# bit-current/DistributedTraining

Measured on AMD Instinct MI355X. Metric: tokens/sec (whole node, all miners), GPT-2-small local-SGD, higher is better.
Workload: dtype bf16; 1 GPU; model=gpt2-small, global_batch=1024, seq_len=64, parallelism=local_sgd_dp1, merge_every=25, optimizer=fused AdamW (lr 5e-4, reference config)

## Files before the change

distributedtraining_amd/ops/__init__.py:

```python

from __future__ import annotations

import math
from typing import Optional

import torch
import torch.nn.functional as F

from . import droprng
from .backend import require_ext, use_hip

__all__ = [
    "layer_norm", "rms_norm", "gelu", "swiglu", "causal_attention",
    "qkv_attention", "linear", "mlp_gelu", "add_layer_norm",
    "add_rms_norm",
    "cross_entropy_loss", "lm_head_ce", "lm_head_loss",
    "embedding_fwd", "check_q_lo", "check_doc_start", "q_lo_inverse",
    "decode_attention", "rope", "adamw_step", "delta_sub", "axpy_",
    "weighted_merge",
    "grad_merge_weights", "has_nan", "l2norm",
    "grad_sumsq_blocks", "grad_sumsq_partials", "step_control",
    "adamw_step_guarded", "lr_schedule",
    "quantize_blockwise_int8", "dequantize_blockwise_int8",
    "topk_compress_blockwise",
    "dropout", "rng_tick",
]


import os as _os

_USE_BGRADB = _os.environ.get("DTA_LT_BGRADB", "0") == "1"

class _LinearFn(torch.autograd.Function):

    @staticmethod
    def forward(ctx, x, w, b):
        x2 = x.reshape(-1, x.shape[-1])
        ctx.save_for_backward(x2, w)
        ctx.has_b = b is not None
        ctx.xshape = x.shape
        ctx.wgrad = getattr(w, "main_grad", None)
        ctx.bgrad = getattr(b, "main_grad", None) if b is not None else None
        y = torch.addmm(b, x2, w.t()) if b is not None else x2.mm(w.t())
        return y.view(*x.shape[:-1], w.shape[0])

    @staticmethod
    def backward(ctx, dy):
        x2, w = ctx.saved_tensors
        dy2 = dy.reshape(-1, dy.shape[-1])
        if dy2.stride(-1) != 1:
            dy2 = dy2.contiguous()
        dx = dy2.mm(w).view(ctx.xshape)
        m = require_ext()
        if _USE_BGRADB and ctx.has_b and ctx.wgrad is not None:
            try:
                db = m.lt_wgrad_bgradb(dy2, x2, ctx.wgrad)
                return dx, None, db
            except RuntimeError:
                pass
        if ctx.wgrad is not None:
            ctx.wgrad.addmm_(dy2.t(), x2)
            dw = None
        else:
            dw = dy2.t().mm(x2)
        db = (_cast_grad(m.colsum(dy2, ctx.bgrad), w.dtype)
              if ctx.has_b else None)
        return dx, dw, db


def linear(x: torch.Tensor, w: torch.Tensor,
           b: Optional[torch.Tensor] = None) -> torch.Tensor:
    if use_hip(x):
        rows = x.numel() // x.shape[-1]
        if rows <= 4 and not torch.is_grad_enabled() and _gemv_wins(rows, w):
            x2 = x.reshape(rows, x.shape[-1])
            if not x2.is_contiguous():
                x2 = x2.contiguous()
            y = require_ext().gemv(
                x2, w, b if b is not None
                else torch.empty(0, dtype=w.dtype, device=w.device))
            return y.view(*x.shape[:-1], w.shape[0])
        return _LinearFn.apply(x, w, b)
    return F.linear(x, w, b)


def _gemv_wins(rows: int, w: torch.Tensor) -> bool:
    if w.shape[1] % 8 != 0:
        return False
    numel = w.shape[0] * w.shape[1]
    return numel < (20_000_000 if rows == 1 else 5_000_000)


_lt_fused_shape_ok: dict = {}


class _FusedMLPFn(torch.autograd.Function):

    @staticmethod
    def forward(ctx, x, w1, b1, w2, b2):
        m = require_ext()
        x2 = x.reshape(-1, x.shape[-1])
        h, aux = m.lt_linear_gelu_fwd(x2.contiguous(), w1, b1)
        y = torch.addmm(b2, h, w2.t())
        ctx.save_for_backward(x2, w1, w2, h, aux)
        ctx.xshape = x.shape
        ctx.w1grad = getattr(w1, "main_grad", None)
        ctx.w2grad = getattr(w2, "main_grad", None)
        ctx.b2grad = getattr(b2, "main_grad", None)
        return y.view(*x.shape[:-1], w2.shape[0])

    @staticmethod
    def backward(ctx, dy):
        m = require_ext()
        x2, w1, w2, h, aux = ctx.saved_tensors
        dy2 = dy.reshape(-1, dy.shape[-1])
        if dy2.stride(-1) != 1:
            dy2 = dy2.contiguous()
        db2 = _cast_grad(m.colsum(dy2, ctx.b2grad), w2.dtype)
        if ctx.w2grad is not None:
            ctx.w2grad.addmm_(dy2.t(), h)
            dw2 = None
        else:
            dw2 = dy2.t().mm(h)
        dh_pre, db1 = m.lt_dgrad_dgelu_bgrad(dy2, w2, aux)
        if ctx.w1grad is not None:
            ctx.w1grad.addmm_(dh_pre.t(), x2)
            dw1 = None
        else:
            dw1 = dh_pre.t().mm(x2)
        dx = dh_pre.mm(w1).view(ctx.xshape)
        return dx, dw1, db1, dw2, db2


_MLP_NODE = _os.environ.get("DTA_MLP_NODE", "1") != "0"


def mlp_node_enable(on: bool) -> bool:
    global _MLP_NODE
    prev, _MLP_NODE = _MLP_NODE, bool(on)
    return prev


class _MLPGeluFn(torch.autograd.Function):

    @staticmethod
    def forward(ctx, x, w1, b1, w2, b2):
        m = require_ext()
        x2 = x.reshape(-1, x.shape[-1])
        pre = torch.addmm(b1, x2, w1.t())
        h = m.gelu_fwd(pre)
        y = torch.addmm(b2, h, w2.t())
        ctx.save_for_backward(x2, w1, w2, pre, h)
        ctx.xshape = x.shape
        ctx.grads = tuple(getattr(t, "main_grad", None)
                          for t in (w1, b1, w2, b2))
        return y.view(*x.shape[:-1], w2.shape[0])

    @staticmethod
    def backward(ctx, dy):
        m = require_ext()
        x2, w1, w2, pre, h = ctx.saved_tensors
        w1g, b1g, w2g, b2g = ctx.grads
        dy2 = dy.reshape(-1, dy.shape[-1])
        if dy2.stride(-1) != 1:
            dy2 = dy2.contiguous()
        dh = dy2.mm(w2)
        if w2g is not None:
            w2g.addmm_(dy2.t(), h)
            dw2 = None
        else:
            dw2 = dy2.t().mm(h)
        db2 = _cast_grad(m.colsum(dy2, b2g), w2.dtype)
        dh_pre, db1 = m.gelu_bwd_colsum(dh, pre, b1g)
        del dh
        dx = dh_pre.mm(w1).view(ctx.xshape)
        if w1g is not None:
            w1g.addmm_(dh_pre.t(), x2)
            dw1 = None
        else:
            dw1 = dh_pre.t().mm(x2)
        return dx, dw1, _cast_grad(db1, w1.dtype), dw2, db2


def mlp_gelu(x: torch.Tensor, w1: torch.Tensor, b1: torch.Tensor,
             w2: torch.Tensor, b2: torch.Tensor) -> torch.Tensor:
    if use_hip(x):
        rows = x.numel() // x.shape[-1]
        if rows <= 4 and not torch.is_grad_enabled():
            return linear(gelu(linear(x, w1, b1)), w2, b2)
        key = (rows, w1.shape[0], w1.shape[1])
        if _lt_fused_shape_ok.get(key, True):
            try:
                out = _FusedMLPFn.apply(x, w1, b1, w2, b2)
                _lt_fused_shape_ok[key] = True
                return out
            except RuntimeError as e:
                import logging
                logging.getLogger(__name__).warning(
                    "hipBLASLt epilogue MLP unavailable at M,N,K=%s (%s); "
                    "composed path", key, e)
                _lt_fused_shape_ok[key] = False
        if _MLP_NODE and all(t.dtype == torch.bfloat16
                             for t in (x, w1, b1, w2, b2)):
            return _MLPGeluFn.apply(x, w1, b1, w2, b2)
        return linear(gelu(linear(x, w1, b1)), w2, b2)
    return F.linear(F.gelu(F.linear(x, w1, b1), approximate="tanh"), w2, b2)


def _empty_like0(t):
    return t.new_empty(0)


def _rng0(t: torch.Tensor) -> torch.Tensor:
    return droprng.counter(t.device)


def _grad_out(fp32_grad, main_grad, dtype):
    if main_grad is not None:
        require_ext().accum_f32_into_bf16(main_grad, fp32_grad)
        return None
    return fp32_grad.to(dtype)


def _cast_grad(fp32_grad, dtype):
    return None if fp32_grad is None else fp32_grad.to(dtype)


def _cpu_drop(t: torch.Tensor, p: float, site: int) -> torch.Tensor:
    keep = droprng.elem_keep_mask(t.numel(), droprng.value(t.device), site, p)
    mask = torch.from_numpy(keep.astype("float32")).reshape(t.shape)
    return t * (mask * droprng.inv_keep(p)).to(t.dtype)


def _norm_fwd(x2, res, w, b, eps, site, p):
    m = require_ext()
    if b is None:
        y, rstd, s = m.rmsnorm_fwd(x2, res, w, eps, _rng0(x2), site, p)
        return y, (rstd,), s
    y, mean, rstd, s = m.layernorm_fwd(x2, res, w, b, eps, _rng0(x2), site, p)
    return y, (mean, rstd), s


def _norm_bwd(dy, ds, x2, w, stats, site, p, wg=None, bg=None):
    m = require_ext()
    if len(stats) == 1:
        dx, dw32, dres = m.rmsnorm_bwd(dy, ds, x2, w, *stats, _rng0(x2),
                                       site, p, wg)
        return dx, dw32, None, dres
    return m.layernorm_bwd(dy, ds, x2, w, *stats, _rng0(x2), site, p, wg, bg)


class _NormFn(torch.autograd.Function):
    @staticmethod
    def forward(ctx, x, w, b, eps):
        x2 = x.contiguous()
        y, stats, _ = _norm_fwd(x2.view(-1, x2.shape[-1]), _empty_like0(x2),
                                w, b, eps, 0, 0.0)
        ctx.save_for_backward(x2, w, *stats)
        ctx.wg = getattr(w, "main_grad", None)
# ... 975 lines not shown
```

distributedtraining_amd/ops/hip/bindings.cpp:

```cpp
#include <torch/extension.h>
#include <ATen/hip/HIPContext.h>

#include <algorithm>
#include <atomic>
#include <vector>

#include "dta_kernels.h"

namespace {

using torch::Tensor;

inline hipStream_t stream() {
  return at::hip::getCurrentHIPStream().stream();
}
inline const bf16_t* bfp(const Tensor& t) {
  return reinterpret_cast<const bf16_t*>(t.data_ptr());
}
inline bf16_t* bfp_mut(Tensor& t) {
  return reinterpret_cast<bf16_t*>(t.data_ptr());
}

void check_bf16(const Tensor& t, const char* name) {
  TORCH_CHECK(t.is_cuda(), name, " must be on GPU");
// ... 271 lines not shown
  }
  TORCH_CHECK(has_part || (max_norm <= 0.0 && !skip_nonfinite),
              "clipping and the non-finite skip need the norm partials");
  TORCH_CHECK(part.numel() <= (int64_t(1) << 30), "too many partials");
  TORCH_CHECK(schedule >= LR_CONSTANT && schedule <= LR_COSINE,
              "unknown schedule");
  TORCH_CHECK(warmup_steps >= 0 && warmup_steps < (int64_t(1) << 31) &&
                  total_steps >= 0 && total_steps < (int64_t(1) << 31),
              "warmup_steps / total_steps out of range");
  TORCH_CHECK(schedule == LR_CONSTANT || total_steps > warmup_steps,
              "linear / cosine need total_steps > warmup_steps");
  launch_step_ctl({has_part ? part.data_ptr<float>() : nullptr,
                   int(part.numel()), ctl_f.data_ptr<float>(),
                   ctl_i.data_ptr<int>(), beta1, beta2, float(max_norm),
                   skip_nonfinite ? 1 : 0, int(schedule), lr_max, min_lr,
                   int(warmup_steps), int(total_steps)},
                  stream());
}
void adamw_step_guarded(Tensor master, Tensor grad, Tensor m, Tensor v,
                        Tensor out_bf16, Tensor ctl_f, Tensor ctl_i,
                        double beta1, double beta2, double eps, double wd) {
  check_f32(master, "master"); check_f32(m, "m"); check_f32(v, "v");
  const bool gb = flat_grad_is_bf16(grad, "grad");
  const int64_t n = master.numel();
  TORCH_CHECK(grad.numel() == n && m.numel() == n && v.numel() == n,
              "master, grad, m and v must have one length");
  TORCH_CHECK(grad.device() == master.device() &&
                  m.device() == master.device() &&
                  v.device() == master.device(), "planes on one device");
  check_ctl(ctl_f, ctl_i, master);
  bf16_t* outp = nullptr;
  if (out_bf16.numel()) {
    check_bf16(out_bf16, "out_bf16");
    TORCH_CHECK(out_bf16.numel() == n && out_bf16.device() == master.device(),
                "out_bf16 must match master");
    outp = bfp_mut(out_bf16);
  }
  launch_adamw_guarded(master.data_ptr<float>(), grad.data_ptr(), gb,
                       m.data_ptr<float>(), v.data_ptr<float>(), outp,
                       ctl_f.data_ptr<float>(), ctl_i.data_ptr<int>(), beta1,
                       beta2, float(eps), float(wd), n, stream());
}

Tensor colsum(Tensor x, OptTensor dst) {
  check_bf16(x, "x");
  TORCH_CHECK(x.dim() == 2 && x.size(1) >= 1, "x must be [rows, cols]");
  const int64_t rows = x.size(0);
  const int cols = int(x.size(1));
  const int stripes = dta_colred_stripes(rows, cols);
  auto f32 = x.options().dtype(torch::kFloat32);
  auto part = torch::empty({stripes, dta_colred_ld(cols)}, f32);
  bf16_t* d = grad_dst(dst, cols, "dst");
  Tensor out = d ? Tensor() : torch::empty({cols}, f32);
  launch_colsum(bfp(x), part.data_ptr<float>(),
                d ? nullptr : out.data_ptr<float>(), d, rows, cols, stripes,
                stream());
  return out;
}

std::vector<Tensor> gelu_bwd_colsum(Tensor dy, Tensor x, OptTensor db_dst,
                                    int64_t stripes_arg) {
  check_bf16(x, "x"); check_bf16(dy, "dy");
  TORCH_CHECK(x.dim() == 2 && dy.sizes() == x.sizes(),
              "dy, x must be [rows, cols]");
  const int64_t rows = x.size(0);
  const int cols = int(x.size(1));
  if (cols % 8 != 0) {
    auto dx = gelu_bwd(dy, x);
    return {dx, colsum(dx, db_dst)};
  }
  const int stripes =
      stripes_arg > 0 ? int(std::min<int64_t>(stripes_arg, 65535))
                      : dta_gelu_colsum_stripes(rows, cols);
  auto f32 = x.options().dtype(torch::kFloat32);
  auto dx = torch::empty_like(x);
  auto part = torch::empty({stripes, cols}, f32);
  bf16_t* d = grad_dst(db_dst, cols, "db_dst");
  Tensor out = d ? Tensor() : torch::empty({cols}, f32);
  launch_gelu_bwd_colsum(bfp(dy), bfp(x), bfp_mut(dx),
                         part.data_ptr<float>(),
                         d ? nullptr : out.data_ptr<float>(), d, rows, cols,
                         stripes, stream());
  return {dx, out};
}

int merge_n_models(int64_t n) {
  TORCH_CHECK(n >= 1 && n <= DTA_MERGE_MAX_MODELS,
              "merge: 1 <= n_models <= ", DTA_MERGE_MAX_MODELS);
  return int(n);
}
int merge_n_segs(const Tensor& offsets) {
  TORCH_CHECK(offsets.dim() == 1 && offsets.numel() >= 2 &&
                  (offsets.scalar_type() == torch::kInt64 ||
                   offsets.scalar_type() == torch::kInt32),
              "offsets must be an int64 or int32 [n_segs + 1] tensor");
  TORCH_CHECK(offsets.numel() <= int64_t(DTA_MERGE_LDS_LIMIT / 8),
              "offsets do not fit the LDS budget of ", DTA_MERGE_LDS_LIMIT,
              " B");
  return int(offsets.numel() - 1);
}
Tensor merge_offsets(const Tensor& offsets, const Tensor& base) {
  return offsets.to(base.device(), torch::kInt64).contiguous();
}
Tensor merge_weights(const Tensor& W, const Tensor& base, int n_models,
                     int n_segs) {
  TORCH_CHECK(W.dim() == 2 && W.size(0) == n_models && W.size(1) == n_segs,
              "W must be [n_models, n_segs]");
  TORCH_CHECK(dta_merge_shmem(n_models, n_segs) <= DTA_MERGE_LDS_LIMIT,
              "offsets + W ([", n_models, ", ", n_segs,
              "]) do not fit the LDS budget of ", DTA_MERGE_LDS_LIMIT, " B");
  return W.to(base.device(), torch::kFloat32).contiguous();
}
void check_plane_f32(const Tensor& t, int64_t P, const char* name) {
  check_f32(t, name);
  TORCH_CHECK(t.numel() == P, name, " must have P elements");
}
int check_deltas_f32(const Tensor& deltas, int64_t P) {
  check_f32(deltas, "deltas");
  TORCH_CHECK(P >= 1 && deltas.dim() == 2 && deltas.size(1) == P,
              "deltas must be [N, P]");
  return merge_n_models(deltas.size(0));
}

void weighted_merge(Tensor base, Tensor deltas, Tensor W, Tensor offsets,
                    Tensor out) {
  const int64_t P = base.numel();
  check_plane_f32(base, P, "base"); check_plane_f32(out, P, "out");
  const int n_models = check_deltas_f32(deltas, P);
  const int n_segs = merge_n_segs(offsets);
  auto Wc = merge_weights(W, base, n_models, n_segs);
  auto offs = merge_offsets(offsets, base);
  launch_weighted_merge(base.data_ptr<float>(), deltas.data_ptr<float>(),
                        Wc.data_ptr<float>(), offs.data_ptr<int64_t>(),
                        n_models, n_segs, P, out.data_ptr<float>(), stream());
}

Tensor grad_w_chunks(const Tensor& offsets, const Tensor& base, int n_segs) {
  auto offs_cpu = offsets.to(torch::kCPU, torch::kInt64).contiguous();
  const int64_t* op = offs_cpu.data_ptr<int64_t>();
  TORCH_CHECK(op[0] == 0 && op[n_segs] == base.numel(),
              "offsets must run from 0 to P");
  for (int j = 0; j < n_segs; ++j)
    TORCH_CHECK(op[j] <= op[j + 1], "offsets must not decrease");
  std::vector<int64_t> chunks;
  constexpr int64_t CH = 1 << 20;
  for (int j = 0; j < n_segs; ++j)
    for (int64_t s0 = op[j]; s0 < op[j + 1]; s0 += CH) {
      chunks.push_back(s0);
      chunks.push_back(std::min(s0 + CH, op[j + 1]));
      chunks.push_back(j);
    }
  return torch::from_blob(chunks.data(), {int64_t(chunks.size())},
                          torch::kInt64)
      .to(base.device());
}

bool check_grad_plane(const Tensor& g, int64_t P) {
  const bool gb = g.scalar_type() == torch::kBFloat16;
  TORCH_CHECK(g.is_cuda() && g.is_contiguous() && g.numel() == P &&
                  (gb || g.scalar_type() == torch::kFloat32),
              "g must be a contiguous bf16/fp32 [P] GPU tensor");
  return gb;
}

Tensor grad_merge_weights(Tensor g, Tensor base, Tensor deltas, Tensor merged,
                          Tensor offsets) {
// ... 693 lines not shown
                     Tensor o_bshd, Tensor lse, double scale, Tensor dq_v,
                     Tensor dk_v, Tensor dv_v, Tensor kvlen, Tensor rng,
                     int64_t site, double p, OptDoc q_lo, OptDoc k_hi) {
  TORCH_CHECK(dk_v.stride(3) == 1 && dv_v.stride(3) == 1,
              "dqkv views need contiguous head_dim");
  auto [dk32, dv32] = attn_bwd_into(dout, q, k, v, o_bshd, lse, scale, kvlen,
                                    rng, site, p, dq_v, dk_v, dv_v, q_lo,
                                    k_hi);
  if (!dk32.defined()) return;
  dk_v.copy_(dk32.permute({0, 2, 1, 3}));
  dv_v.copy_(dv32.permute({0, 2, 1, 3}));
}

Tensor attn_decode(Tensor q, Tensor kc, Tensor vc, int64_t kv_len,
                   double scale, Tensor len_dev) {
  check_bf16(q, "q"); check_bf16(kc, "kcache"); check_bf16(vc, "vcache");
  TORCH_CHECK(q.dim() == 3 && kc.dim() == 4, "q [B,H,D], cache [B,Hk,L,D]");
  const int B = int(q.size(0)), H = int(q.size(1)), hd = int(q.size(2));
  const int Hk = int(kc.size(1));
  TORCH_CHECK(hd == 64 || hd == 128, "decode head dim must be 64/128");
  TORCH_CHECK(H % Hk == 0 && kv_len <= kc.size(2), "bad cache geometry");
  const int* lp = nullptr;
  if (len_dev.numel()) {
    TORCH_CHECK(len_dev.scalar_type() == torch::kInt32 && len_dev.is_cuda(),
                "len_dev must be an int32 GPU scalar");
    lp = len_dev.data_ptr<int>();
  }
  auto o = torch::empty_like(q);
  launch_attn_decode(bfp(q), bfp(kc), bfp(vc), bfp_mut(o), B, H, H / Hk,
                     int(kv_len), lp, hd, kc.stride(0), kc.stride(1),
                     float(scale), stream());
  return o;
}

Tensor mfma_selftest_16(Tensor A, Tensor B) {
  check_bf16(A, "A"); check_bf16(B, "B");
  auto D = torch::zeros({16, 16}, A.options().dtype(torch::kFloat32));
  launch_mfma_probe_16(bfp(A), bfp(B), D.data_ptr<float>(), stream());
  return D;
}
Tensor mfma_selftest_32(Tensor A, Tensor B) {
  check_bf16(A, "A"); check_bf16(B, "B");
  auto D = torch::zeros({32, 32}, A.options().dtype(torch::kFloat32));
  launch_mfma_probe_32(bfp(A), bfp(B), D.data_ptr<float>(), stream());
  return D;
}

}

void register_lt_fused(pybind11::module& m);

PYBIND11_MODULE(TORCH_EXTENSION_NAME, m) {
  register_lt_fused(m);
  m.def("layernorm_fwd", &layernorm_fwd);
  namespace py = pybind11;
  m.def("layernorm_bwd", &layernorm_bwd, py::arg("dy"), py::arg("ds"),
        py::arg("x"), py::arg("w"), py::arg("mean"), py::arg("rstd"),
        py::arg("rng"), py::arg("site"), py::arg("p"),
        py::arg("dw_dst") = py::none(), py::arg("db_dst") = py::none());
  m.def("rmsnorm_fwd", &rmsnorm_fwd);
  m.def("rmsnorm_bwd", &rmsnorm_bwd, py::arg("dy"), py::arg("ds"),
        py::arg("x"), py::arg("w"), py::arg("rstd"), py::arg("rng"),
        py::arg("site"), py::arg("p"), py::arg("dw_dst") = py::none());
  m.def("gelu_fwd", &gelu_fwd);
  m.def("gelu_bwd", &gelu_bwd);
  m.def("gelu_bwd_colsum", &gelu_bwd_colsum, py::arg("dy"), py::arg("x"),
        py::arg("db_dst") = py::none(), py::arg("stripes") = 0);
  m.def("swiglu_fwd", &swiglu_fwd);
  m.def("swiglu_bwd", &swiglu_bwd);
  m.def("dropout_apply", &dropout_apply);
  m.def("rng_tick", &rng_tick);
  m.def("accum_f32_into_bf16", &accum_f32_into_bf16);
  m.def("delta_sub", &delta_sub);
  m.def("axpy", &axpy);
  m.def("has_nan", &has_nan);
  m.def("l2norm_sq", &l2norm_sq);
  m.def("adamw_step", &adamw_step);
  m.def("adamw_tick", &adamw_tick);
  m.def("grad_sumsq_blocks", &grad_sumsq_blocks);
  m.def("grad_sumsq_partials", &grad_sumsq_partials);
  m.def("step_control", &step_control);
  m.def("adamw_step_guarded", &adamw_step_guarded);
  m.def("colsum", &colsum, py::arg("x"), py::arg("dst") = py::none());
  m.def("weighted_merge", &weighted_merge);
  m.def("grad_merge_weights", &grad_merge_weights);
  m.def("weighted_merge_packed", &weighted_merge_packed);
  m.def("grad_merge_weights_packed", &grad_merge_weights_packed);
  m.def("axpy_packed", &axpy_packed);
  m.def("quantize_int8", &quantize_int8, py::arg("x"), py::arg("base"),
        py::arg("block"), py::arg("topk_k") = 0,
        py::arg("residual_in") = py::none(),
        py::arg("residual_out") = py::none());
  m.def("ce_fwd", &ce_fwd);
  m.def("ce_bwd", &ce_bwd);
  m.def("ce_fwd_bwd", &ce_fwd_bwd, pybind11::arg("logits"),
        pybind11::arg("targets"), pybind11::arg("ignore_index"),
        pybind11::arg("inv_count_dev"), pybind11::arg("max_rows") = 0,
        pybind11::arg("lds_row") = false);
  m.def("ce_chunk", &ce_chunk);
  m.def("ce_finalize", &ce_finalize);
  m.def("head_loss_fwd", &head_loss_fwd);
  m.def("embedding_fwd", &embedding_fwd, py::arg("ids"), py::arg("wte"),
        py::arg("wpe"), py::arg("pos"), py::arg("doc_start") = py::none());
  m.def("embedding_bwd", &embedding_bwd, py::arg("dy"), py::arg("ids"),
        py::arg("vocab"), py::arg("npos"),
        py::arg("doc_start") = py::none());
  m.def("kv_append", &kv_append);
  m.def("i32_inc", &i32_inc);
  m.def("gemv", &gemv);
  m.def("rope_fwd", &rope_fwd);
  m.def("rope_bwd", &rope_bwd);
  m.def("attn_fwd", &attn_fwd, py::arg("q"), py::arg("k"), py::arg("v"),
        py::arg("scale"), py::arg("kvlen"), py::arg("rng"), py::arg("site"),
        py::arg("p"), py::arg("q_lo") = py::none());
  m.def("attn_bwd", &attn_bwd, py::arg("dout"), py::arg("q"), py::arg("k"),
        py::arg("v"), py::arg("o_bshd"), py::arg("lse"), py::arg("scale"),
        py::arg("kvlen"), py::arg("rng"), py::arg("site"), py::arg("p"),
        py::arg("q_lo") = py::none(), py::arg("k_hi") = py::none());
  m.def("attn_bwd_packed", &attn_bwd_packed, py::arg("dout"), py::arg("q"),
        py::arg("k"), py::arg("v"), py::arg("o_bshd"), py::arg("lse"),
        py::arg("scale"), py::arg("dq_v"), py::arg("dk_v"), py::arg("dv_v"),
        py::arg("kvlen"), py::arg("rng"), py::arg("site"), py::arg("p"),
        py::arg("q_lo") = py::none(), py::arg("k_hi") = py::none());
  m.def("attn_bwd_fused_enable", &attn_bwd_fused_enable);
  m.def("attn_bwd_fused_calls", &attn_bwd_fused_calls);
  m.def("attn_decode", &attn_decode);
  m.def("mfma_selftest_16", &mfma_selftest_16);
  m.def("mfma_selftest_32", &mfma_selftest_32);
}
```

distributedtraining_amd/ops/hip/dta_kernels.h:

```cpp
#pragma once

#include <hip/hip_runtime.h>
#include <cmath>
#include <cstdint>
#include <cstdlib>

using bf16_t = unsigned short;

struct DropParams {
  const unsigned long long* rng = nullptr;
  unsigned long long site = 0;
  unsigned int thr16 = 0;
  float inv_keep = 1.0f;
};
inline void dta_drop_quantize(double p, DropParams& d) {
  const double full = 65536.0;
  d.thr16 = (unsigned int)std::fmin(std::ceil(p * full), full - 1.0);
  d.inv_keep = float(full / (full - double(d.thr16)));
}

void launch_gelu_fwd(const bf16_t* x, bf16_t* y, int64_t n, hipStream_t s);
void launch_gelu_bwd(const bf16_t* dy, const bf16_t* x, bf16_t* dx, int64_t n,
                     hipStream_t s);
void launch_gelu_fwd_f32(const float* x, float* y, int64_t n, hipStream_t s);
// ... 153 lines not shown
}
inline int dta_norm_bwd_grid(int64_t rows) {
  int64_t want = (rows + DTA_NORM_ROW_WAVES - 1) / DTA_NORM_ROW_WAVES;
  return int(want < 4096 ? (want > 0 ? want : 1) : 4096);
}
inline int dta_norm_bwd_stripes(int64_t rows, int cols) {
  return dta_norm_fused_dwdb(cols) ? dta_norm_bwd_grid(rows)
                                   : dta_colred_stripes(rows, cols);
}
constexpr int DTA_NORM_FWD_MAX_COLS = 8192;
constexpr int DTA_NORM_BWD_MAX_COLS = 4096;
struct NormFwdArgs {
  const bf16_t *x, *res;
  bf16_t* sum_out;
  const bf16_t *w, *b;
  bf16_t* y;
  float *mean, *rstd;
  int64_t rows;
  int cols;
  float eps;
  DropParams drop;
  bool rms;
};
struct NormBwdArgs {
  const bf16_t *dy, *ds, *x, *w;
  const float *mean, *rstd;
  bf16_t *dx, *dres;
  float *dw, *db, *pdw, *pdb;
  bf16_t *dw_dst, *db_dst;
  int stripes;
  int64_t rows;
  int cols;
  DropParams drop;
  bool rms;
};
void launch_norm_fwd(const NormFwdArgs& a, hipStream_t s);
void launch_norm_bwd(const NormBwdArgs& a, hipStream_t s);

void launch_ce_fwd(const bf16_t* logits, const int64_t* targets,
                   int64_t rows, int64_t vocab, int64_t ignore_index,
                   float* lse, float* loss_sum, int* count, hipStream_t s);
void launch_ce_bwd(const bf16_t* logits, const int64_t* targets,
                   const float* lse, float scale, const float* scale_p,
                   int64_t ignore_index, int64_t v0, bool nt,
                   bf16_t* dlogits, int64_t rows, int64_t vocab,
                   hipStream_t s);
void launch_ce_fwd_bwd(bf16_t* logits, const int64_t* targets, int64_t rows,
                       int64_t vocab, int64_t ignore_index,
                       const float* inv_count, float* lse, float* loss_sum,
                       int* count, int max_blocks, hipStream_t s);
bool launch_ce_fwd_bwd_lds(bf16_t* logits, const int64_t* targets,
                           int64_t rows, int64_t vocab, int64_t ignore_index,
                           const float* inv_count, float* lse,
                           float* loss_sum, int* count, int n_cu,
                           int64_t lds_limit, hipStream_t s);
inline int dta_ce_fwd_bwd_blocks(int64_t vocab, int n_cu) {
  const int64_t fit = (int64_t(128) << 20) / (2 * (vocab > 0 ? vocab : 1));
  const int64_t lo = n_cu > 0 ? n_cu : 1;
  return int(fit < lo ? lo : (fit > 4096 ? 4096 : fit));
}
void launch_ce_chunk(const bf16_t* chunk, int64_t ld, int64_t rows,
                     int64_t cols, const int64_t* targets, int64_t v0,
                     float* tlogit, float* m_run, float* s_run,
                     hipStream_t s);
void launch_ce_finalize(const int64_t* targets, const float* m_run,
                        const float* s_run, const float* tlogit,
                        int64_t rows, int64_t ignore_index, float* lse,
                        float* loss_sum, int* count, hipStream_t s);

constexpr int DTA_HEAD_LOSS_TILE = 128;
inline int dta_head_loss_nsplit(int64_t T, int64_t V, int cus) {
  const int64_t rb = (T + DTA_HEAD_LOSS_TILE - 1) / DTA_HEAD_LOSS_TILE;
  const int64_t nt = (V + DTA_HEAD_LOSS_TILE - 1) / DTA_HEAD_LOSS_TILE;
  int64_t ns = (4 * int64_t(cus) + rb - 1) / (rb > 0 ? rb : 1);
  if (ns > nt) ns = nt;
  if (ns > 65535) ns = 65535;
  return int(ns < 1 ? 1 : ns);
}
void launch_head_loss(const bf16_t* x, const bf16_t* w,
                      const int64_t* targets, int64_t T, int64_t V, int K,
                      int nsplit, float* ws_m, float* ws_s, float* tlogit,
                      float* m_run, float* s_run, hipStream_t s);

void launch_embedding_fwd(const int64_t* ids, const bf16_t* wte,
                          const bf16_t* wpe, bf16_t* out, int64_t n_tok,
                          int seq_len, int dim, bool has_wpe,
                          const int* pos_p, const int* doc_start,
                          hipStream_t s);
inline int dta_doc_dwpe_stripes(int64_t B, int seq, int dim) {
  return dta_colred_stripes(B, seq * dim);
}
void launch_embedding_dwpe_doc(const bf16_t* dy, const int* doc_start,
                               float* part, float* out, int64_t B, int seq,
                               int dim, int stripes, hipStream_t s);
void launch_kv_append(const bf16_t* kn, const bf16_t* vn, int64_t knb,
                      bf16_t* kc, bf16_t* vc, const int* pos_p, int B,
                      int Hk, int D, int64_t cb, int64_t ch, hipStream_t s);
void launch_i32_inc(int* p, hipStream_t s);
void launch_embedding_bwd(const bf16_t* dy, const int64_t* ids,
                          float* dwte_f32, float* dwpe_f32, int64_t n_tok,
                          int seq_len, int dim, bool has_wpe, hipStream_t s);
void launch_f32_to_bf16(const float* x, bf16_t* y, int64_t n, hipStream_t s);

void launch_gemv(const bf16_t* x, const bf16_t* w, const bf16_t* bias,
                 bf16_t* y, int M, int64_t N, int K, hipStream_t s);

void launch_rope(const bf16_t* x, const float* cos_t, const float* sin_t,
                 bf16_t* y, int64_t bh, int seq, int hd, bool backward,
                 const int* pos_p, hipStream_t s);

struct AttnStride { int64_t batch, head, seq; };
struct AttnGeom {
  int B, H, grp, seq, hd;
  float scale;
  AttnStride q, k, v, o;
  AttnStride dout, dq;
  AttnStride dkv;
  const int* kvlen = nullptr;
  DropParams drop;
  const int* q_lo = nullptr;
  const int* k_hi = nullptr;
};
void launch_attn_fwd(const bf16_t* q, const bf16_t* k, const bf16_t* v,
                     bf16_t* o, float* lse, const AttnGeom& geo,
                     hipStream_t s);
void launch_attn_bwd_dq(const bf16_t* dout, const bf16_t* q, const bf16_t* k,
                        const bf16_t* v, const bf16_t* o, const float* lse,
                        float* delta, bf16_t* dq, const AttnGeom& geo,
                        hipStream_t s);
void launch_attn_bwd_dkv(const bf16_t* dout, const bf16_t* q,
                         const bf16_t* k, const bf16_t* v, const float* lse,
                         const float* delta, float* dk32, float* dv32,
                         bf16_t* dk, bf16_t* dv, const AttnGeom& geo,
                         hipStream_t s);
inline bool dta_attn_bwd_fused_shape(const AttnGeom& geo) {
  return geo.seq <= 64 && geo.grp == 1 && (geo.hd == 32 || geo.hd == 64);
}
inline bool dta_attn_bwd_fused_default() {
  static const bool en = [] {
    const char* e = ::getenv("DTA_ATTN_BWD_FUSED");
    return !(e && e[0] == '0');
  }();
  return en;
}
void launch_attn_bwd_fused(const bf16_t* dout, const bf16_t* q,
                           const bf16_t* k, const bf16_t* v, const bf16_t* o,
                           const float* lse, bf16_t* dq, bf16_t* dk,
                           bf16_t* dv, const AttnGeom& geo, hipStream_t s);

void launch_attn_decode(const bf16_t* q, const bf16_t* kc, const bf16_t* vc,
                        bf16_t* o, int B, int H, int grp, int kvlen,
                        const int* len_p, int hd, int64_t cb, int64_t ch,
                        float scale, hipStream_t s);

void launch_mfma_probe_32(const bf16_t* A, const bf16_t* B, float* D,
                          hipStream_t s);
void launch_mfma_probe_16(const bf16_t* A, const bf16_t* B, float* D,
                          hipStream_t s);
```

setup.py:

```python

import os

from setuptools import find_packages, setup

os.environ.setdefault("PYTORCH_ROCM_ARCH", "gfx950")

from torch.utils.cpp_extension import BuildExtension, CUDAExtension

SRC = [
    "distributedtraining_amd/ops/hip/bindings.cpp",
    "distributedtraining_amd/ops/hip/lt_fused.cpp",
    "distributedtraining_amd/ops/hip/elementwise.hip",
    "distributedtraining_amd/ops/hip/adamw.hip",
    "distributedtraining_amd/ops/hip/norms.hip",
    "distributedtraining_amd/ops/hip/ce.hip",
    "distributedtraining_amd/ops/hip/head_loss.hip",
    "distributedtraining_amd/ops/hip/embedding.hip",
    "distributedtraining_amd/ops/hip/rope.hip",
    "distributedtraining_amd/ops/hip/gemv.hip",
    "distributedtraining_amd/ops/hip/merge.hip",
    "distributedtraining_amd/ops/hip/attention.hip",
]

setup(
    name="distributedtraining_amd",
    version="0.2.0",
    packages=find_packages(include=["distributedtraining_amd*"]),
    ext_modules=[
        CUDAExtension(
            name="distributedtraining_amd._dta_hip",
            sources=SRC,
            libraries=["hipblaslt"],
            extra_compile_args={
                "cxx": ["-O3", "-std=c++17"],
                "nvcc": ["-O3", "-std=c++17", "--offload-arch=gfx950"],
            },
        )
    ],
    cmdclass={"build_ext": BuildExtension},
)
```

Before: 915,800 tokens/s.

## Add split-K MFMA weight-gradient kernel with fused bias reduction

Adds a custom HIP kernel that computes weight gradients dW += dy^T x using split-K over the token dimension. Partial fp32 results go to a slab, and a fold kernel sums them into the bf16 main_grad. The kernel also computes the bias column sum through extra MFMAs with a ones vector, so the separate colsum launch goes away. It is routed automatically for the GPT-2-small linear and MLP shapes at T of 32768 or 65536. The aim is to beat hipBLASLt addmm on tall-skinny K-dominant GEMMs. The cost is an extra fp32 slab allocation and write/read traffic.

Measured after the change: 971,100 tokens/s, median of 6. 1.06x the previous value.

```diff
diff --git a/distributedtraining_amd/ops/__init__.py b/distributedtraining_amd/ops/__init__.py
--- a/distributedtraining_amd/ops/__init__.py
+++ b/distributedtraining_amd/ops/__init__.py
@@ -31,6 +31,41 @@
 
 _USE_BGRADB = _os.environ.get("DTA_LT_BGRADB", "0") == "1"
 
+_WGRAD = _os.environ.get("DTA_WGRAD", "auto")
+if _WGRAD not in ("0", "1"):
+    _WGRAD = "auto"
+
+
+def wgrad_route(mode: str) -> str:
+    global _WGRAD
+    if mode not in ("0", "1", "auto"):
+        raise ValueError(f"wgrad_route: {mode!r}")
+    prev, _WGRAD = _WGRAD, mode
+    return prev
+
+
+_WGRAD_WINS: frozenset = frozenset(
+    (T, out, inp) for T in (65536, 32768)
+    for out, inp in ((2304, 768), (768, 768), (3072, 768), (768, 3072)))
+
+
+def _wgrad_wins(T: int, out: int, inp: int) -> bool:
+    return (T, out, inp) in _WGRAD_WINS
+
+
+def _wgrad_accum(m, dy2, x2, wgrad, bgrad, want_bias):
+    if _WGRAD == "0" or wgrad is None or dy2.dtype != torch.bfloat16:
+        return False, None
+    if _WGRAD == "auto" and not _wgrad_wins(
+            dy2.shape[0], dy2.shape[1], x2.shape[1]):
+        return False, None
+    if not (wgrad.is_contiguous() and m.wgrad.supported(dy2, x2)):
+        return False, None
+    db32 = m.wgrad.bias(dy2, x2, wgrad, bgrad if want_bias else None,
+                        want_bias and bgrad is None)
+    return True, (db32 if want_bias and bgrad is None else None)
+
+
 class _LinearFn(torch.autograd.Function):
 
     @staticmethod
@@ -58,6 +93,9 @@
                 return dx, None, db
             except RuntimeError:
                 pass
+        done, db32 = _wgrad_accum(m, dy2, x2, ctx.wgrad, ctx.bgrad, ctx.has_b)
+        if done:
+            return dx, None, _cast_grad(db32, w.dtype)
         if ctx.wgrad is not None:
             ctx.wgrad.addmm_(dy2.t(), x2)
             dw = None
@@ -165,16 +203,23 @@
         if dy2.stride(-1) != 1:
             dy2 = dy2.contiguous()
         dh = dy2.mm(w2)
-        if w2g is not None:
-            w2g.addmm_(dy2.t(), h)
-            dw2 = None
+        done, db32 = _wgrad_accum(m, dy2, h, w2g, b2g, True)
+        if done:
+            dw2, db2 = None, _cast_grad(db32, w2.dtype)
         else:
-            dw2 = dy2.t().mm(h)
-        db2 = _cast_grad(m.colsum(dy2, b2g), w2.dtype)
+            if w2g is not None:
+                w2g.addmm_(dy2.t(), h)
+                dw2 = None
+            else:
+                dw2 = dy2.t().mm(h)
+            db2 = _cast_grad(m.colsum(dy2, b2g), w2.dtype)
         dh_pre, db1 = m.gelu_bwd_colsum(dh, pre, b1g)
         del dh
         dx = dh_pre.mm(w1).view(ctx.xshape)
-        if w1g is not None:
+        done, _ = _wgrad_accum(m, dh_pre, x2, w1g, None, False)
+        if done:
+            dw1 = None
+        elif w1g is not None:
             w1g.addmm_(dh_pre.t(), x2)
             dw1 = None
         else:
diff --git a/distributedtraining_amd/ops/hip/bindings.cpp b/distributedtraining_amd/ops/hip/bindings.cpp
--- a/distributedtraining_amd/ops/hip/bindings.cpp
+++ b/distributedtraining_amd/ops/hip/bindings.cpp
@@ -377,6 +377,74 @@
                          d ? nullptr : out.data_ptr<float>(), d, rows, cols,
                          stripes, stream());
   return {dx, out};
+}
+
+const char* wgrad_reject(const Tensor& dy, const Tensor& x) {
+  if (!(dy.is_cuda() && x.is_cuda() && dy.device() == x.device()))
+    return "dy and x must be on one GPU";
+  if (dy.scalar_type() != torch::kBFloat16 ||
+      x.scalar_type() != torch::kBFloat16)
+    return "dy and x must be bf16";
+  if (dy.dim() != 2 || x.dim() != 2 || dy.size(0) != x.size(0))
+    return "dy must be [T, out] and x [T, in]";
+  const int64_t T = dy.size(0), out = dy.size(1), in = x.size(1);
+  if (T < 1 || T >= (int64_t(1) << 31)) return "T out of range";
+  if (out < DTA_WGRAD_BM || out % DTA_WGRAD_BM != 0 || in < DTA_WGRAD_BN ||
+      in % DTA_WGRAD_BN != 0 || out * in >= (int64_t(1) << 31))
+    return "out / in must be multiples of the tile";
+  if (dy.stride(1) != 1 || x.stride(1) != 1) return "unit column stride";
+  const int64_t lda = T > 1 ? dy.stride(0) : out, ldb = T > 1 ? x.stride(0) : in;
+  if (lda < out || ldb < in || lda % 8 != 0 || ldb % 8 != 0 ||
+      lda >= (int64_t(1) << 25) || ldb >= (int64_t(1) << 25))
+    return "row strides must be >= the width, % 8 == 0 and < 2^25";
+  if (reinterpret_cast<uintptr_t>(dy.data_ptr()) % 16 != 0 ||
+      reinterpret_cast<uintptr_t>(x.data_ptr()) % 16 != 0)
+    return "16-byte aligned operands";
+  return nullptr;
+}
+bool wgrad_supported(Tensor dy, Tensor x) { return !wgrad_reject(dy, x); }
+std::vector<int64_t> wgrad_tile() {
+  return {DTA_WGRAD_BM, DTA_WGRAD_BN, DTA_WGRAD_BK};
+}
+int64_t wgrad_nsplit(int64_t T, int64_t out, int64_t in) {
+  return dta_wgrad_nsplit(
+      T, out, in, at::cuda::getCurrentDeviceProperties()->multiProcessorCount);
+}
+
+Tensor wgrad_bias(Tensor dy, Tensor x, Tensor dw, OptTensor db, bool bias_f32,
+                  int64_t nsplit) {
+  const char* why = wgrad_reject(dy, x);
+  TORCH_CHECK(!why, "wgrad_bias: ", why ? why : "");
+  const int64_t T = dy.size(0), out = dy.size(1), in = x.size(1);
+  check_bf16(dw, "dw");
+  TORCH_CHECK(dw.device() == dy.device() && dw.dim() == 2 &&
+                  dw.size(0) == out && dw.size(1) == in,
+              "dw must be a contiguous bf16 [out, in] view on dy's device");
+  bf16_t* dbp = grad_dst(db, out, "db");
+  TORCH_CHECK(!dbp || db->device() == dy.device(), "db must be on dy's device");
+  TORCH_CHECK(nsplit >= 0, "nsplit must be >= 0");
+  const int ns = nsplit == 0 ? int(wgrad_nsplit(T, out, in))
+                             : int(std::min<int64_t>(nsplit, 1024));
+  const bool bias = dbp || bias_f32;
+  const auto f32 = dy.options().dtype(torch::kFloat32);
+  auto slab = torch::empty({int64_t(ns), out, in}, f32);
+  Tensor bpart = bias ? torch::empty({int64_t(ns), out}, f32) : Tensor();
+  Tensor bout = (bias && !dbp) ? torch::empty({out}, f32) : Tensor();
+  WgradArgs a;
+  a.dy = bfp(dy); a.x = bfp(x);
+  a.ld_dy = T > 1 ? dy.stride(0) : out;
+  a.ld_x = T > 1 ? x.stride(0) : in;
+  a.T = T; a.out = int(out); a.in = int(in); a.nsplit = ns;
+  a.slab = slab.data_ptr<float>();
+  a.bpart = bias ? bpart.data_ptr<float>() : nullptr;
+  a.dw = bfp_mut(dw);
+  a.db = dbp;
+  a.bout = bout.defined() ? bout.data_ptr<float>() : nullptr;
+  launch_wgrad(a, stream());
+  const hipError_t err = hipGetLastError();
+  TORCH_CHECK(err == hipSuccess, "wgrad launch failed: ",
+              hipGetErrorString(err));
+  return bout;
 }
 
 int merge_n_models(int64_t n) {
@@ -1236,6 +1304,13 @@
   m.def("step_control", &step_control);
   m.def("adamw_step_guarded", &adamw_step_guarded);
   m.def("colsum", &colsum, py::arg("x"), py::arg("dst") = py::none());
+  py::module_ wg = m.def_submodule("wgrad", "split-K weight gradient");
+  wg.def("bias", &wgrad_bias, py::arg("dy"), py::arg("x"), py::arg("dw"),
+         py::arg("db") = py::none(), py::arg("bias_f32") = false,
+         py::arg("nsplit") = 0);
+  wg.def("supported", &wgrad_supported);
+  wg.def("tile", &wgrad_tile);
+  wg.def("nsplit", &wgrad_nsplit);
   m.def("weighted_merge", &weighted_merge);
   m.def("grad_merge_weights", &grad_merge_weights);
   m.def("weighted_merge_packed", &weighted_merge_packed);
diff --git a/distributedtraining_amd/ops/hip/dta_kernels.h b/distributedtraining_amd/ops/hip/dta_kernels.h
--- a/distributedtraining_amd/ops/hip/dta_kernels.h
+++ b/distributedtraining_amd/ops/hip/dta_kernels.h
@@ -259,6 +259,26 @@
                       int nsplit, float* ws_m, float* ws_s, float* tlogit,
                       float* m_run, float* s_run, hipStream_t s);
 
+constexpr int DTA_WGRAD_BM = 256;
+constexpr int DTA_WGRAD_BN = 128;
+constexpr int DTA_WGRAD_BK = 32;
+inline int dta_wgrad_nsplit(int64_t T, int64_t out, int64_t in, int cus) {
+  const int64_t tiles = (out / DTA_WGRAD_BM) * (in / DTA_WGRAD_BN);
+  const int64_t ksteps = (T + DTA_WGRAD_BK - 1) / DTA_WGRAD_BK;
+  int64_t ns = 2 * int64_t(cus) / (tiles > 0 ? tiles : 1);
+  if (ns > ksteps) ns = ksteps;
+  return int(ns < 1 ? 1 : ns);
+}
+struct WgradArgs {
+  const bf16_t *dy, *x;
+  int64_t ld_dy, ld_x, T;
+  int out, in, nsplit;
+  float *slab, *bpart;
+  bf16_t *dw, *db;
+  float* bout;
+};
+void launch_wgrad(const WgradArgs& a, hipStream_t s);
+
 void launch_embedding_fwd(const int64_t* ids, const bf16_t* wte,
                           const bf16_t* wpe, bf16_t* out, int64_t n_tok,
                           int seq_len, int dim, bool has_wpe,
diff --git a/distributedtraining_amd/ops/hip/wgrad.hip b/distributedtraining_amd/ops/hip/wgrad.hip
--- /dev/null
+++ b/distributedtraining_amd/ops/hip/wgrad.hip
@@ -0,0 +1,224 @@
+#include "dta_common.h"
+#include "dta_kernels.h"
+
+namespace {
+
+constexpr int BM = DTA_WGRAD_BM, BN = DTA_WGRAD_BN, BK = DTA_WGRAD_BK;
+constexpr int WG_THREADS = 512;
+static_assert(BM == 256 && BN == 128 && BK == 32, "wave layout and staging");
+
+constexpr int A_S = BM * 2 + 32, A_G = 8 * A_S + 128;
+constexpr int B_S = BN * 2 + 32, B_G = 8 * B_S + 128;
+constexpr int A_BYTES = (BK / 8) * A_G;
+constexpr int B_BYTES = (BK / 8) * B_G;
+constexpr int BUF_BYTES = A_BYTES + B_BYTES;
+static_assert(A_S % 256 == 32 && B_S % 256 == 32, "bank spread of rows");
+static_assert(A_G % 256 == 128 && B_G % 256 == 128, "bank spread of groups");
+
+typedef __attribute__((address_space(3))) s16x4 lds_s16x4;
+
+DEV bf16x8 tr_frag(const char* p, int row_stride) {
+  const s16x4 lo = __builtin_amdgcn_ds_read_tr16_b64_v4i16((lds_s16x4*)p);
+  const s16x4 hi =
+      __builtin_amdgcn_ds_read_tr16_b64_v4i16((lds_s16x4*)(p + 4 * row_stride));
+  return as_bf16x8(__builtin_shufflevector(lo, hi, 0, 1, 2, 3, 4, 5, 6, 7));
+}
+
+template <bool BIAS>
+__global__ __launch_bounds__(WG_THREADS)
+__attribute__((amdgpu_waves_per_eu(4, 4))) void wgrad_k(
+    const ushort* __restrict__ dy, int64_t ld_dy, const ushort* __restrict__ x,
+    int64_t ld_x, int64_t T, int out, int in, int nsplit,
+    float* __restrict__ slab, float* __restrict__ bpart) {
+  __shared__ __attribute__((aligned(16))) char lds[2 * BUF_BYTES];
+
+  const int tid = threadIdx.x;
+  const int lane = tid & 63;
+  const int wid = __builtin_amdgcn_readfirstlane(tid >> 6);
+  const int wm = wid >> 1, wn = wid & 1;
+  const int fr = lane & 15, fq = lane >> 4;
+
+  const int tiles_n = in / BN;
+  const int tiles = (out / BM) * tiles_n;
+  const int nwg = gridDim.x;
+  const int bq = nwg >> 3, br = nwg & 7;
+  const int xcd = blockIdx.x & 7;
+  const int wgid = (xcd < br ? xcd * (bq + 1) : br * (bq + 1) + (xcd - br) * bq) +
+                   (blockIdx.x >> 3);
+  const int slice = wgid / tiles, tile = wgid - slice * tiles;
+  const int tm = tile / tiles_n, tn = tile - tm * tiles_n;
+  const int m0 = tm * BM, n0 = tn * BN;
+
+  const int64_t ksteps = (T + BK - 1) / BK;
+  const int64_t k_begin = ksteps * slice / nsplit;
+  const int64_t k_end = ksteps * (slice + 1) / nsplit;
+  const int nsteps = int(k_end - k_begin);
+
+  const int ac = tid & 31, ar = tid >> 5;
+  const int bc = tid & 15, br_ = tid >> 4;
+  const char* abase = reinterpret_cast<const char*>(dy + m0);
+  const char* bbase = reinterpret_cast<const char*>(x + n0);
+  const unsigned a_col = ac * 16, b_col = bc * 16;
+  const unsigned a_ldb = unsigned(ld_dy) * 2, b_ldb = unsigned(ld_x) * 2;
+  const int a_st0 = (ar & 7) * A_S + (ar >> 3) * A_G + ac * 16;
+  const int a_st1 = a_st0 + 2 * A_G;
+  const int b_st = A_BYTES + (br_ & 7) * B_S + (br_ >> 3) * B_G + bc * 16;
+
+  const int tq = fr >> 2, tp = fr & 3;
+  const int a_rd = tq * A_S + fq * A_G + (wm * 64 + 4 * tp) * 2;
+  const int b_rd = A_BYTES + tq * B_S + fq * B_G + (wn * 64 + 4 * tp) * 2;
+
+  const bool bias_wave = BIAS && tn == 0 && wn == 0;
+
+  f32x4 acc[4][4];
+#pragma unroll
+  for (int i = 0; i < 4; ++i)
+#pragma unroll
+    for (int n = 0; n < 4; ++n) acc[i][n] = f32x4{0.f, 0.f, 0.f, 0.f};
+  f32x4 bacc = {0.f, 0.f, 0.f, 0.f};
+
+  s16x8 ga0, ga1, gb;
+  const s16x8 zero8 = {0, 0, 0, 0, 0, 0, 0, 0};
+  auto gload = [&](int64_t kstep) {
+    const int64_t t0 = kstep * BK;
+    const char* arow = abase + t0 * ld_dy * 2;
+    const char* brow = bbase + t0 * ld_x * 2;
+    if (t0 + BK <= T) {
+      ga0 = *reinterpret_cast<const s16x8*>(arow + (ar * a_ldb + a_col));
+      ga1 = *reinterpret_cast<const s16x8*>(arow + ((ar + 16) * a_ldb + a_col));
+      gb = *reinterpret_cast<const s16x8*>(brow + (br_ * b_ldb + b_col));
+    } else {
+      const int rem = int(T - t0);
+      const int r0 = ar < rem ? ar : rem - 1;
+      const int r1 = ar + 16 < rem ? ar + 16 : rem - 1;
+      const int rb = br_ < rem ? br_ : rem - 1;
+      ga0 = *reinterpret_cast<const s16x8*>(arow + (r0 * a_ldb + a_col));
+      ga1 = *reinterpret_cast<const s16x8*>(arow + (r1 * a_ldb + a_col));
+      gb = *reinterpret_cast<const s16x8*>(brow + (rb * b_ldb + b_col));
+      if (ar >= rem) ga0 = zero8;
+      if (ar + 16 >= rem) ga1 = zero8;
+      if (br_ >= rem) gb = zero8;
+    }
+  };
+  auto lds_write = [&](char* buf) {
+    *reinterpret_cast<s16x8*>(buf + a_st0) = ga0;
+    *reinterpret_cast<s16x8*>(buf + a_st1) = ga1;
+    *reinterpret_cast<s16x8*>(buf + b_st) = gb;
+  };
+
+  if (nsteps > 0) {
+    gload(k_begin);
+    lds_write(lds);
+  }
+  __syncthreads();
+
+  for (int it = 0; it < nsteps; ++it) {
+    const bool more = it + 1 < nsteps;
+    if (more) gload(k_begin + it + 1);
+
+    const char* buf = lds + (it & 1) * BUF_BYTES;
+    bf16x8 a[4], b[4];
+#pragma unroll
+    for (int i = 0; i < 4; ++i) {
+      a[i] = tr_frag(buf + a_rd + i * 32, A_S);
+      b[i] = tr_frag(buf + b_rd + i * 32, B_S);
+    }
+#pragma unroll
+    for (int i = 0; i < 4; ++i)
+#pragma unroll
+      for (int n = 0; n < 4; ++n) acc[i][n] = mfma_bf16(a[i], b[n], acc[i][n]);
+    if (BIAS && bias_wave) {
+      int sel = tq;
+      asm volatile("" : "+v"(sel));
+#pragma unroll
+      for (int i = 0; i < 4; ++i) {
+        const short one = sel == i ? short(0x3F80) : short(0);
+        const s16x8 o = {one, one, one, one, one, one, one, one};
+        bacc = mfma_bf16(as_bf16x8(o), a[i], bacc);
+      }
+    }
+
+    if (more) lds_write(lds + ((it + 1) & 1) * BUF_BYTES);
+    __syncthreads();
+  }
+
+  float* sp = slab + int64_t(slice) * out * int64_t(in) +
+              int64_t(m0 + wm * 64 + 4 * fq) * in + n0 + wn * 64 + fr;
+#pragma unroll
+  for (int i = 0; i < 4; ++i)
+#pragma unroll
+    for (int j = 0; j < 4; ++j)
+#pragma unroll
+      for (int n = 0; n < 4; ++n)
+        sp[int64_t(i * 16 + j) * in + n * 16] = acc[i][n][j];
+  if (BIAS && bias_wave)
+    bpart[int64_t(slice) * out + m0 + wm * 64 + fq * 16 + fr] = bacc[0];
+}
+
+DEV float fold1(const float* __restrict__ p, int64_t stride, int ns) {
+  float s = p[0];
+#pragma unroll 4
+  for (int i = 1; i < ns; ++i) s += p[int64_t(i) * stride];
+  return s;
+}
+
+template <bool VEC>
+__global__ __launch_bounds__(256) void wgrad_fold_k(
+    const float* __restrict__ slab, int ns, int64_t n_w, ushort* __restrict__ dw,
+    int wblocks, const float* __restrict__ bpart, int n_b,
+    ushort* __restrict__ db, float* __restrict__ bout) {
+  if (int(blockIdx.x) < wblocks) {
+    if (VEC) {
+      const int64_t e = (int64_t(blockIdx.x) * 256 + threadIdx.x) * 4;
+      if (e < n_w) {
+        f32x4 s = *reinterpret_cast<const f32x4*>(slab + e);
+#pragma unroll 4
+        for (int i = 1; i < ns; ++i)
+          s += *reinterpret_cast<const f32x4*>(slab + int64_t(i) * n_w + e);
+        s16x4 d = *reinterpret_cast<const s16x4*>(dw + e);
+#pragma unroll
+        for (int j = 0; j < 4; ++j)
+          d[j] = short(f2bf(bf2f(ushort(d[j])) + s[j]));
+        *reinterpret_cast<s16x4*>(dw + e) = d;
+      }
+    } else {
+      const int64_t e = int64_t(blockIdx.x) * 256 + threadIdx.x;
+      if (e < n_w) dw[e] = f2bf(bf2f(dw[e]) + fold1(slab + e, n_w, ns));
+    }
+  } else {
+    const int e = (int(blockIdx.x) - wblocks) * 256 + threadIdx.x;
+    if (e < n_b) {
+      const float s = fold1(bpart + e, n_b, ns);
+      if (db) db[e] = f2bf(bf2f(db[e]) + s);
+      else bout[e] = s;
+    }
+  }
+}
+
+}
+
+void launch_wgrad(const WgradArgs& a, hipStream_t s) {
+  const int tiles = (a.out / BM) * (a.in / BN);
+  const unsigned grid = unsigned(tiles) * unsigned(a.nsplit);
+  if (a.bpart)
+    wgrad_k<true><<<grid, WG_THREADS, 0, s>>>(a.dy, a.ld_dy, a.x, a.ld_x, a.T,
+                                              a.out, a.in, a.nsplit, a.slab,
+                                              a.bpart);
+  else
+    wgrad_k<false><<<grid, WG_THREADS, 0, s>>>(a.dy, a.ld_dy, a.x, a.ld_x, a.T,
+                                               a.out, a.in, a.nsplit, a.slab,
+                                               nullptr);
+  const int64_t n_w = int64_t(a.out) * a.in;
+  const bool vec = reinterpret_cast<uintptr_t>(a.dw) % 8 == 0;
+  const int wblocks = int((n_w + (vec ? 1024 : 256) - 1) / (vec ? 1024 : 256));
+  const int n_b = a.bpart ? a.out : 0;
+  const unsigned fgrid = unsigned(wblocks + (n_b + 255) / 256);
+  if (vec)
+    wgrad_fold_k<true><<<fgrid, 256, 0, s>>>(a.slab, a.nsplit, n_w, a.dw,
+                                             wblocks, a.bpart, n_b, a.db,
+                                             a.bout);
+  else
+    wgrad_fold_k<false><<<fgrid, 256, 0, s>>>(a.slab, a.nsplit, n_w, a.dw,
+                                              wblocks, a.bpart, n_b, a.db,
+                                              a.bout);
+}
diff --git a/setup.py b/setup.py
--- a/setup.py
+++ b/setup.py
@@ -15,6 +15,7 @@
     "distributedtraining_amd/ops/hip/norms.hip",
     "distributedtraining_amd/ops/hip/ce.hip",
     "distributedtraining_amd/ops/hip/head_loss.hip",
+    "distributedtraining_amd/ops/hip/wgrad.hip",
     "distributedtraining_amd/ops/hip/embedding.hip",
     "distributedtraining_amd/ops/hip/rope.hip",
     "distributedtraining_amd/ops/hip/gemv.hip",
```
